# Eddie-Wang1120/Eddie-Wang-Hackathon2023

Measured on AMD Instinct MI355X. Metric: decode tokens/s, whole job (encoder + cross-KV + language-ID + prefill + greedy decode), Whisper large-v2 int8 weight-only + int8 KV; rtf reported beside it, higher is better.
Workload: dtype f16

## Files before the change

eddie-wang-hackathon2023_amd/csrc/attn_encoder.hip:

```cpp
#include <stdlib.h>

#include <type_traits>

#include "common.h"
#include "kernels.h"

namespace wm {

constexpr int KT_KEYS = 64;
constexpr int AROW = 128;
constexpr int KV_TILE = KT_KEYS * AROW;

template <int QB, bool PERSIST = false>
__global__ __launch_bounds__(256, 2) void attn_encoder_kernel(AttnEncParams p) {
    __shared__ __attribute__((aligned(1024))) unsigned char smem[4 * KV_TILE];
    auto sK = [&](int b) { return smem + b * 2 * KV_TILE; };
    auto sV = [&](int b) { return smem + b * 2 * KV_TILE + KV_TILE; };

    const int tid = threadIdx.x, lane = tid & 63, wid = tid >> 6;
    const int g = lane >> 4, li = lane & 15;
    const int C = p.H * 64;
    const int nx = (p.T + 64 * QB - 1) / (64 * QB), n_heads = p.H * p.B;
    const int n_items = 8 * ((n_heads + 7) / 8) * nx;
    int item = blockIdx.x;
    do {
    const int hh = ((item >> 3) / nx) * 8 + (item & 7), bx = (item >> 3) % nx;
    if (hh < n_heads) {
    const int h = hh % p.H, b = hh / p.H;
    const int q_base = bx * (64 * QB) + wid * (16 * QB);
    const h16* base = p.qkv + (size_t)b * p.T * p.ld;

    half8v qf[QB][2];
#pragma unroll
    for (int qb = 0; qb < QB; ++qb) {
        int qrow = q_base + qb * 16 + li;
        if (qrow > p.T - 1) qrow = p.T - 1;
#pragma unroll
        for (int s = 0; s < 2; ++s)
            qf[qb][s] = *(const half8v*)(base + (size_t)qrow * p.ld + h * 64 + s * 32 + g * 8);
    }

    auto load_kv = [&](int tile, int buf) {
#pragma unroll
        for (int i = 0; i < 2; ++i) {
            const int piece = wid + 4 * i;
            const int r = piece * 8 + (lane >> 3);
            int key = tile * KT_KEYS + r;
            if (key > p.T - 1) key = p.T - 1;
            const h16* row = base + (size_t)key * p.ld + h * 64 + (((lane & 7) ^ ((r >> 1) & 7)) * 8);
            __builtin_amdgcn_global_load_lds((const __attribute__((address_space(1))) void*)(row + C),
                                             (__attribute__((address_space(3))) void*)(sK(buf) + piece * 1024), 16, 0, 0);
            __builtin_amdgcn_global_load_lds((const __attribute__((address_space(1))) void*)(row + 2 * C),
                                             (__attribute__((address_space(3))) void*)(sV(buf) + piece * 1024), 16, 0, 0);
        }
    };

    float4v o[4][QB];
#pragma unroll
    for (int db = 0; db < 4; ++db)
#pragma unroll
        for (int qb = 0; qb < QB; ++qb) o[db][qb] = float4v{0.f, 0.f, 0.f, 0.f};
    float m_run[QB], l_run[QB];
#pragma unroll
    for (int qb = 0; qb < QB; ++qb) { m_run[qb] = -INFINITY; l_run[qb] = 0.f; }

    const int ntiles = (p.T + KT_KEYS - 1) / KT_KEYS;
    load_kv(0, 0);
    asm volatile("s_waitcnt vmcnt(0)" ::: "memory");
    __syncthreads();

    const int k_swz = (li >> 1) & 7;
    const int k_off0 = li * AROW + ((g ^ k_swz) << 4), k_off1 = li * AROW + (((g + 4) ^ k_swz) << 4);
    const int v_row = 4 * g + (li >> 2), v_swz = (v_row >> 1) & 7;
    const int v_base = v_row * AROW + (li & 1) * 8, v_chunk = (li & 3) >> 1;

    auto tile_body = [&](int t, auto TAIL_) {
        constexpr bool TAIL = decltype(TAIL_)::value;
        const int cur = t & 1;
        if (t + 1 < ntiles) load_kv(t + 1, cur ^ 1);

        float4v sacc[4][QB];
#pragma unroll
        for (int kb = 0; kb < 4; ++kb) {
            const half8v k0 = *(const half8v*)(sK(cur) + k_off0 + kb * 16 * AROW);
            const half8v k1 = *(const half8v*)(sK(cur) + k_off1 + kb * 16 * AROW);
#pragma unroll
            for (int qb = 0; qb < QB; ++qb) {
                float4v a = float4v{0.f, 0.f, 0.f, 0.f};
                a = __builtin_amdgcn_mfma_f32_16x16x32_f16(k0, qf[qb][0], a, 0, 0, 0);
                a = __builtin_amdgcn_mfma_f32_16x16x32_f16(k1, qf[qb][1], a, 0, 0, 0);
                sacc[kb][qb] = a;
            }
        }
        const int key0 = t * KT_KEYS + 4 * g;
        half8v pf[2][QB];
        constexpr float LOG2E = 1.4426950408889634f;
        float mx[QB];
#pragma unroll
        for (int qb = 0; qb < QB; ++qb) {
            float m = -INFINITY;
#pragma unroll
            for (int kb = 0; kb < 4; ++kb)
#pragma unroll
                for (int r = 0; r < 4; ++r) {
                    if (TAIL && key0 + 16 * kb + r >= p.T) sacc[kb][qb][r] = -INFINITY;
                    m = fmaxf(m, sacc[kb][qb][r]);
                }
            mx[qb] = m;
        }
        {
            float o16[QB];
#pragma unroll
            for (int qb = 0; qb < QB; ++qb) o16[qb] = __shfl_xor(mx[qb], 16);
#pragma unroll
            for (int qb = 0; qb < QB; ++qb) mx[qb] = fmaxf(mx[qb], o16[qb]);
            float o32[QB];
#pragma unroll
            for (int qb = 0; qb < QB; ++qb) o32[qb] = __shfl_xor(mx[qb], 32);
#pragma unroll
            for (int qb = 0; qb < QB; ++qb) mx[qb] = fmaxf(mx[qb], o32[qb]);
        }
        float mL[QB], alpha[QB];
        bool moved = false;
#pragma unroll
        for (int qb = 0; qb < QB; ++qb) {
            const float m_old = m_run[qb];
            const float m_new = fmaxf(m_old, r16(mx[qb]));
            float mn = __fmul_rn(m_new, LOG2E), mo = __fmul_rn(m_old, LOG2E);
            asm volatile("" : "+v"(mn), "+v"(mo));
            mL[qb] = mn;
            alpha[qb] = __builtin_amdgcn_exp2f(__fsub_rn(mo, mL[qb]));
            moved |= (m_new != m_old);
            m_run[qb] = m_new;
        }
        const bool any_moved = __builtin_amdgcn_ballot_w64(moved) != 0;
#pragma unroll
        for (int qb = 0; qb < QB; ++qb) {
            float ps = 0.f;
            const half2v one2 = {(h16)1.0f, (h16)1.0f};
#pragma unroll
            for (int kb = 0; kb < 4; ++kb)
#pragma unroll
                for (int r = 0; r < 4; r += 2) {
                    const half2v s2 = __builtin_convertvector(float2v{sacc[kb][qb][r], sacc[kb][qb][r + 1]}, half2v);
                    const float p0 = __builtin_amdgcn_exp2f(__fmaf_rn((float)s2[0], LOG2E, -mL[qb]));
                    const float p1 = __builtin_amdgcn_exp2f(__fmaf_rn((float)s2[1], LOG2E, -mL[qb]));
                    const half2v p2 = __builtin_convertvector(float2v{p0, p1}, half2v);
                    ps = __builtin_amdgcn_fdot2(p2, one2, ps, false);
                    pf[kb >> 1][qb][(kb & 1) * 4 + r] = p2[0];
                    pf[kb >> 1][qb][(kb & 1) * 4 + r + 1] = p2[1];
                }
            l_run[qb] = __fmaf_rn(l_run[qb], alpha[qb], ps);
        }
        if (any_moved) {
#pragma unroll
            for (int qb = 0; qb < QB; ++qb)
#pragma unroll
                for (int db = 0; db < 4; ++db) o[db][qb] *= alpha[qb];
        }
#pragma unroll
        for (int c = 0; c < 2; ++c) {
#pragma unroll
            for (int db = 0; db < 4; ++db) {
                const unsigned char* va = sV(cur) + v_base + (c * 32) * AROW + (((2 * db + v_chunk) ^ v_swz) << 4);
                const short4r lo = __builtin_amdgcn_ds_read_tr16_b64_v4i16(
                    (__attribute__((address_space(3))) short4r*)(va));
                const short4r hi = __builtin_amdgcn_ds_read_tr16_b64_v4i16(
                    (__attribute__((address_space(3))) short4r*)(va + 16 * AROW));
                half8v vf;
                const half4v l4 = __builtin_bit_cast(half4v, lo), h4 = __builtin_bit_cast(half4v, hi);
#pragma unroll
                for (int j = 0; j < 4; ++j) { vf[j] = l4[j]; vf[4 + j] = h4[j]; }
#pragma unroll
                for (int qb = 0; qb < QB; ++qb)
                    o[db][qb] = __builtin_amdgcn_mfma_f32_16x16x32_f16(vf, pf[c][qb], o[db][qb], 0, 0, 0);
            }
        }
        asm volatile("s_waitcnt vmcnt(0)" ::: "memory");
        __syncthreads();
    };
    for (int t = 0; t + 1 < ntiles; ++t) tile_body(t, std::false_type{});
    if (p.T % KT_KEYS != 0) tile_body(ntiles - 1, std::true_type{}); else tile_body(ntiles - 1, std::false_type{});

#pragma unroll
    for (int qb = 0; qb < QB; ++qb) {
        const int qrow = q_base + qb * 16 + li;
        float l = l_run[qb];
        l += __shfl_xor(l, 16);
        l += __shfl_xor(l, 32);
        if (qrow >= p.T) continue;
        const float inv = 1.0f / l;
        h16* dst = p.out + ((size_t)b * p.T + qrow) * p.ldo + h * 64;
#pragma unroll
        for (int db = 0; db < 4; ++db) {
            half4v w;
#pragma unroll
            for (int r = 0; r < 4; ++r) {
                float t = o[db][qb][r] * inv;
                asm volatile("" : "+v"(t));
                w[r] = (h16)t;
            }
            *(half4v*)(dst + db * 16 + g * 4) = w;
        }
    }
    }
    item += gridDim.x;
    } while (PERSIST && item < n_items);
}

int launch_attn_encoder(const AttnEncParams& p, hipStream_t stream) {
    WM_REQUIRE(p.T >= 1 && p.H >= 1 && p.B >= 1, "attn_encoder: bad shape");
    WM_REQUIRE(p.ld % 8 == 0 && p.ldo % 4 == 0, "attn_encoder: leading dimensions must keep 16-byte alignment");
    static const int lab_wgs = lab_env_int("WM_ATTN_MAX_WGS", 0);
    const int max_wgs = p.max_wgs > 0 ? p.max_wgs : lab_wgs;
    const int heads8 = 8 * ((p.H * p.B + 7) / 8);
    if (p.T > 128 && max_wgs > 0 && max_wgs < ((p.T + 255) / 256) * p.H * p.B) {
        hipLaunchKernelGGL((attn_encoder_kernel<4, true>), dim3(max_wgs >= 8 ? max_wgs / 8 * 8 : max_wgs), dim3(256), 0, stream, p);
    } else if (p.T > 128) {
        hipLaunchKernelGGL(attn_encoder_kernel<4>, dim3(heads8 * ((p.T + 255) / 256)), dim3(256), 0, stream, p);
    } else {
        hipLaunchKernelGGL(attn_encoder_kernel<2>, dim3(heads8 * ((p.T + 127) / 128)), dim3(256), 0, stream, p);
    }
    WM_LAUNCH_CHECK(stream, "attn_encoder");
    return 0;
}

}
```

eddie-wang-hackathon2023_amd/csrc/common.h:

```cpp
#pragma once
#include <hip/hip_runtime.h>
#include <hip/hip_fp16.h>
#include <stdint.h>
#include <stddef.h>

namespace wm {

typedef _Float16 h16;
typedef _Float16 half2v __attribute__((ext_vector_type(2)));
typedef float float2v __attribute__((ext_vector_type(2)));
typedef _Float16 half4v __attribute__((ext_vector_type(4)));
typedef _Float16 half8v __attribute__((ext_vector_type(8)));
typedef float float4v __attribute__((ext_vector_type(4)));
typedef float float16v __attribute__((ext_vector_type(16)));
typedef short short4r __attribute__((__vector_size__(4 * sizeof(short))));
typedef unsigned int u32x4 __attribute__((ext_vector_type(4)));

constexpr int WAVE = 64;

void set_error(const char* fmt, ...);
#define WM_CHECK_HIP(expr)                                                                  \
    do {                                                                                    \
        hipError_t _e = (expr);                                                             \
        if (_e != hipSuccess) {                                                             \
            wm::set_error("%s failed: %s (%s:%d)", #expr, hipGetErrorString(_e), __FILE__,  \
                          __LINE__);                                                        \
            return 2;                                                                       \
        }                                                                                   \
    } while (0)
#define WM_REQUIRE(cond, ...)                                                               \
    do {                                                                                    \
        if (!(cond)) {                                                                      \
            wm::set_error(__VA_ARGS__);                                                     \
            return 1;                                                                       \
        }                                                                                   \
    } while (0)
int post_launch_check(hipStream_t s, const char* what);
#define WM_LAUNCH_CHECK(stream, what)                                                       \
    do {                                                                                    \
        int _r = wm::post_launch_check(stream, what);                                       \
        if (_r) return _r;                                                                  \
    } while (0)

int lab_env_int(const char* name, int dflt);
const char* lab_env_str(const char* name);

__device__ __forceinline__ float mul_rn(float a, float b) {
    float r = a * b;
    asm volatile("" : "+v"(r));
    return r;
}
__device__ __forceinline__ float f32_as_is(float v) {
    asm volatile("" : "+v"(v));
    return v;
}
template <int CTRL>
__device__ __forceinline__ float wave_dpp(float v) {
    return __builtin_bit_cast(float, __builtin_amdgcn_update_dpp(0, __builtin_bit_cast(int, v), CTRL, 0xf, 0xf, true));
}
#define WM_SWAP_GUARD "s_nop 7\n\ts_nop 7\n\ts_nop 2\n\t"
__device__ __forceinline__ void wave_swap32(int& x, int& y) {
    asm volatile(WM_SWAP_GUARD "v_mov_b32 %1, %0\n\ts_nop 1\n\tv_permlane32_swap_b32 %0, %1\n\ts_nop 1" : "+v"(x), "=&v"(y));
}
__device__ __forceinline__ void wave_swap16(int& x, int& y) {
    asm volatile(WM_SWAP_GUARD "v_mov_b32 %1, %0\n\ts_nop 1\n\tv_permlane16_swap_b32 %0, %1\n\ts_nop 1" : "+v"(x), "=&v"(y));
}
__device__ __forceinline__ float wave_add_xor16(float v) { int x = __builtin_bit_cast(int, v), y; wave_swap16(x, y); return __builtin_bit_cast(float, x) + __builtin_bit_cast(float, y); }
__device__ __forceinline__ float wave_add_xor32(float v) { int x = __builtin_bit_cast(int, v), y; wave_swap32(x, y); return __builtin_bit_cast(float, x) + __builtin_bit_cast(float, y); }
__device__ __forceinline__ float wave_max_xor16(float v) { int x = __builtin_bit_cast(int, v), y; wave_swap16(x, y); return fmaxf(__builtin_bit_cast(float, x), __builtin_bit_cast(float, y)); }
__device__ __forceinline__ float wave_max_xor32(float v) { int x = __builtin_bit_cast(int, v), y; wave_swap32(x, y); return fmaxf(__builtin_bit_cast(float, x), __builtin_bit_cast(float, y)); }
__device__ __forceinline__ float wave_sum(float v) {
    int x = __builtin_bit_cast(int, v), y;
    wave_swap32(x, y);
    v = __builtin_bit_cast(float, x) + __builtin_bit_cast(float, y);
    x = __builtin_bit_cast(int, v);
    wave_swap16(x, y);
    v = __builtin_bit_cast(float, x) + __builtin_bit_cast(float, y);
    v += wave_dpp<0x128>(v);
    v += wave_dpp<0x124>(v);
    v += wave_dpp<0x4E>(v);
    v += wave_dpp<0xB1>(v);
    return v;
}
__device__ __forceinline__ float wave_sum_pre_mfma(float v) {
    int x = __builtin_bit_cast(int, v), y;
    asm volatile("v_mov_b32 %1, %0\n\ts_nop 1\n\tv_permlane32_swap_b32 %0, %1\n\ts_nop 1" : "+v"(x), "=&v"(y));
    v = __builtin_bit_cast(float, x) + __builtin_bit_cast(float, y);
    x = __builtin_bit_cast(int, v);
    asm volatile("v_mov_b32 %1, %0\n\ts_nop 1\n\tv_permlane16_swap_b32 %0, %1\n\ts_nop 1" : "+v"(x), "=&v"(y));
    v = __builtin_bit_cast(float, x) + __builtin_bit_cast(float, y);
    v += wave_dpp<0x128>(v);
    v += wave_dpp<0x124>(v);
    v += wave_dpp<0x4E>(v);
    v += wave_dpp<0xB1>(v);
    return v;
}
__device__ __forceinline__ float wave_sum_nomfma(float v) { return wave_sum_pre_mfma(v); }
#define WM_X8_STEP(SWAP)                                                                                                         \
    int x0 = __builtin_bit_cast(int, v[0]), x1 = __builtin_bit_cast(int, v[1]), x2 = __builtin_bit_cast(int, v[2]),              \
        x3 = __builtin_bit_cast(int, v[3]), x4 = __builtin_bit_cast(int, v[4]), x5 = __builtin_bit_cast(int, v[5]),              \
        x6 = __builtin_bit_cast(int, v[6]), x7 = __builtin_bit_cast(int, v[7]), y0, y1, y2, y3, y4, y5, y6, y7;                  \
    asm volatile("v_mov_b32 %8, %0\n\tv_mov_b32 %9, %1\n\tv_mov_b32 %10, %2\n\tv_mov_b32 %11, %3\n\t"                            \
                 "v_mov_b32 %12, %4\n\tv_mov_b32 %13, %5\n\tv_mov_b32 %14, %6\n\tv_mov_b32 %15, %7\n\ts_nop 1\n\t"                   \
                 SWAP " %0, %8\n\t" SWAP " %1, %9\n\t" SWAP " %2, %10\n\t" SWAP " %3, %11\n\t"                                    \
                 SWAP " %4, %12\n\t" SWAP " %5, %13\n\t" SWAP " %6, %14\n\t" SWAP " %7, %15\n\ts_nop 1"                            \
                 : "+v"(x0), "+v"(x1), "+v"(x2), "+v"(x3), "+v"(x4), "+v"(x5), "+v"(x6), "+v"(x7),                               \
                   "=&v"(y0), "=&v"(y1), "=&v"(y2), "=&v"(y3), "=&v"(y4), "=&v"(y5), "=&v"(y6), "=&v"(y7));                      \
    v[0] = __builtin_bit_cast(float, x0) + __builtin_bit_cast(float, y0); v[1] = __builtin_bit_cast(float, x1) + __builtin_bit_cast(float, y1);   \
    v[2] = __builtin_bit_cast(float, x2) + __builtin_bit_cast(float, y2); v[3] = __builtin_bit_cast(float, x3) + __builtin_bit_cast(float, y3);   \
    v[4] = __builtin_bit_cast(float, x4) + __builtin_bit_cast(float, y4); v[5] = __builtin_bit_cast(float, x5) + __builtin_bit_cast(float, y5);   \
    v[6] = __builtin_bit_cast(float, x6) + __builtin_bit_cast(float, y6); v[7] = __builtin_bit_cast(float, x7) + __builtin_bit_cast(float, y7);
__device__ __forceinline__ void wave_add_xor16_x8_nomfma(float* v) { WM_X8_STEP("v_permlane16_swap_b32") }
__device__ __forceinline__ void wave_add_xor32_x8_nomfma(float* v) { WM_X8_STEP("v_permlane32_swap_b32") }
#undef WM_X8_STEP
__device__ __forceinline__ float wave_max_nomfma(float v) {
    int x = __builtin_bit_cast(int, v), y;
    asm volatile("v_mov_b32 %1, %0\n\ts_nop 1\n\tv_permlane32_swap_b32 %0, %1\n\ts_nop 1" : "+v"(x), "=&v"(y));
    v = fmaxf(__builtin_bit_cast(float, x), __builtin_bit_cast(float, y));
    x = __builtin_bit_cast(int, v);
    asm volatile("v_mov_b32 %1, %0\n\ts_nop 1\n\tv_permlane16_swap_b32 %0, %1\n\ts_nop 1" : "+v"(x), "=&v"(y));
    v = fmaxf(__builtin_bit_cast(float, x), __builtin_bit_cast(float, y));
    v = fmaxf(v, wave_dpp<0x128>(v));
    v = fmaxf(v, wave_dpp<0x124>(v));
    v = fmaxf(v, wave_dpp<0x4E>(v));
    v = fmaxf(v, wave_dpp<0xB1>(v));
    return v;
}
__device__ __forceinline__ float wave_max(float v) {
    int x = __builtin_bit_cast(int, v), y;
    wave_swap32(x, y);
    v = fmaxf(__builtin_bit_cast(float, x), __builtin_bit_cast(float, y));
    x = __builtin_bit_cast(int, v);
    wave_swap16(x, y);
    v = fmaxf(__builtin_bit_cast(float, x), __builtin_bit_cast(float, y));
    v = fmaxf(v, wave_dpp<0x128>(v));
    v = fmaxf(v, wave_dpp<0x124>(v));
    v = fmaxf(v, wave_dpp<0x4E>(v));
    v = fmaxf(v, wave_dpp<0xB1>(v));
    return v;
}
__device__ __forceinline__ void lane_rows_swap16(uint32_t& a, uint32_t& b) {
    asm volatile("s_nop 1\n\tv_permlane16_swap_b32 %0, %1\n\ts_nop 1" : "+v"(a), "+v"(b));
}
__device__ __forceinline__ float r16(float x) { return (float)(h16)x; }
__device__ __forceinline__ float r16_f32(float x) { asm("" : "+v"(x)); return (float)(h16)x; }

__device__ __forceinline__ float fast_erf(float x) {
    const float ax = fabsf(x);
    const float t = __builtin_amdgcn_rcpf(1.0f + 0.3275911f * ax);
    const float poly = t * (0.254829592f + t * (-0.284496736f + t * (1.421413741f + t * (-1.453152027f + t * 1.061405429f))));
    const float e = __builtin_amdgcn_exp2f(ax * (ax * -1.4426950408889634f));
    return copysignf(1.0f - poly * e, x);
}
__device__ __forceinline__ float gelu_erf(float x) { return 0.5f * x * (1.0f + fast_erf(x * 0.70710678118654752f)); }
__device__ __forceinline__ float2v gelu_erf2(float2v x) {
    const float2v xs = x * 0.70710678118654752f;
    const float2v ax = {fabsf(xs[0]), fabsf(xs[1])};
    const float2v d = 1.0f + 0.3275911f * ax;
    const float2v t = {__builtin_amdgcn_rcpf(d[0]), __builtin_amdgcn_rcpf(d[1])};
    const float2v poly = t * (0.254829592f + t * (-0.284496736f + t * (1.421413741f + t * (-1.453152027f + t * 1.061405429f))));
    const float2v a2 = ax * (ax * -1.4426950408889634f);
    const float2v e = {__builtin_amdgcn_exp2f(a2[0]), __builtin_amdgcn_exp2f(a2[1])};
    const float2v m = 1.0f - poly * e;
    const float2v erf = {copysignf(m[0], xs[0]), copysignf(m[1], xs[1])};
    return 0.5f * x * (1.0f + erf);
}
__device__ __forceinline__ float gelu_tanh(float x) {
    return 0.5f * x * (1.0f + tanhf(0.7978845608028654f * (x + 0.044715f * x * x * x)));
}

__device__ __forceinline__ void cvt_s8x4_f16x4(uint32_t w, half2v& lo, half2v& hi) {
    uint32_t u = w ^ 0x80808080u;
    uint32_t a = __builtin_amdgcn_perm(0x64646464u, u, 0x07010700u);
    uint32_t b = __builtin_amdgcn_perm(0x64646464u, u, 0x07030702u);
    const half2v k = {(h16)1152.0f, (h16)1152.0f};
    lo = __builtin_bit_cast(half2v, a) - k;
    hi = __builtin_bit_cast(half2v, b) - k;
}

}
```

Measured before the change: 16420.

## Prefetch next persistent item and skip dead tail tiles in encoder attention

Restructures the encoder flash-attention kernel so a persistent workgroup prefetches the next item's Q and first K/V tile during the last tile of the current item, removing the drain-and-reload bubble between items. It also skips MFMA and softmax work for key blocks beyond T in the tail tile and for query blocks beyond T in partial tiles. Shuffle-based row reductions are replaced with permlane16/32 swap inline-asm helpers. This adds template variants and register pressure, and the cross-item double-buffer parity logic is easy to get wrong.

```diff
diff --git a/eddie-wang-hackathon2023_amd/csrc/attn_encoder.hip b/eddie-wang-hackathon2023_amd/csrc/attn_encoder.hip
--- a/eddie-wang-hackathon2023_amd/csrc/attn_encoder.hip
+++ b/eddie-wang-hackathon2023_amd/csrc/attn_encoder.hip
@@ -10,6 +10,11 @@
 constexpr int KT_KEYS = 64;
 constexpr int AROW = 128;
 constexpr int KV_TILE = KT_KEYS * AROW;
+
+#ifndef WM_ATTN_OPT
+#define WM_ATTN_OPT 15
+#endif
+constexpr bool OPT_TAIL = WM_ATTN_OPT & 1, OPT_PARTQ = WM_ATTN_OPT & 2, OPT_SWAP = WM_ATTN_OPT & 4, OPT_NEXT = WM_ATTN_OPT & 8;
 
 template <int QB, bool PERSIST = false>
 __global__ __launch_bounds__(256, 2) void attn_encoder_kernel(AttnEncParams p) {
@@ -22,32 +27,35 @@
     const int C = p.H * 64;
     const int nx = (p.T + 64 * QB - 1) / (64 * QB), n_heads = p.H * p.B;
     const int n_items = 8 * ((n_heads + 7) / 8) * nx;
-    int item = blockIdx.x;
-    do {
-    const int hh = ((item >> 3) / nx) * 8 + (item & 7), bx = (item >> 3) % nx;
-    if (hh < n_heads) {
-    const int h = hh % p.H, b = hh / p.H;
-    const int q_base = bx * (64 * QB) + wid * (16 * QB);
-    const h16* base = p.qkv + (size_t)b * p.T * p.ld;
+    auto head_of = [&](int it) { return ((it >> 3) / nx) * 8 + (it & 7); };
+    auto live_item = [&](int it) {
+        while (it < n_items && head_of(it) >= n_heads) it += gridDim.x;
+        return it;
+    };
+    auto head_cols = [&](int it) { const int hh = head_of(it); return p.qkv + (size_t)(hh / p.H) * p.T * p.ld + (hh % p.H) * 64; };
+    auto query_base = [&](int it) { return ((it >> 3) % nx) * (64 * QB) + wid * (16 * QB); };
 
     half8v qf[QB][2];
-#pragma unroll
-    for (int qb = 0; qb < QB; ++qb) {
-        int qrow = q_base + qb * 16 + li;
-        if (qrow > p.T - 1) qrow = p.T - 1;
-#pragma unroll
-        for (int s = 0; s < 2; ++s)
-            qf[qb][s] = *(const half8v*)(base + (size_t)qrow * p.ld + h * 64 + s * 32 + g * 8);
-    }
-
-    auto load_kv = [&](int tile, int buf) {
+    auto load_q = [&](int it) __attribute__((always_inline)) {
+        const h16* cols = head_cols(it);
+        const int q_base = query_base(it);
+#pragma unroll
+        for (int qb = 0; qb < QB; ++qb) {
+            int qrow = q_base + qb * 16 + li;
+            if (qrow > p.T - 1) qrow = p.T - 1;
+#pragma unroll
+            for (int s = 0; s < 2; ++s)
+                qf[qb][s] = *(const half8v*)(cols + (size_t)qrow * p.ld + s * 32 + g * 8);
+        }
+    };
+    auto load_kv = [&](const h16* cols, int tile, int buf) __attribute__((always_inline)) {
 #pragma unroll
         for (int i = 0; i < 2; ++i) {
             const int piece = wid + 4 * i;
             const int r = piece * 8 + (lane >> 3);
             int key = tile * KT_KEYS + r;
             if (key > p.T - 1) key = p.T - 1;
-            const h16* row = base + (size_t)key * p.ld + h * 64 + (((lane & 7) ^ ((r >> 1) & 7)) * 8);
+            const h16* row = cols + (size_t)key * p.ld + (((lane & 7) ^ ((r >> 1) & 7)) * 8);
             __builtin_amdgcn_global_load_lds((const __attribute__((address_space(1))) void*)(row + C),
                                              (__attribute__((address_space(3))) void*)(sK(buf) + piece * 1024), 16, 0, 0);
             __builtin_amdgcn_global_load_lds((const __attribute__((address_space(1))) void*)(row + 2 * C),
@@ -55,6 +63,21 @@
         }
     };
 
+    const int ntiles = (p.T + KT_KEYS - 1) / KT_KEYS;
+    int item = live_item(blockIdx.x);
+    if (item >= n_items) return;
+    int buf0 = 0;
+    load_q(item);
+    load_kv(head_cols(item), 0, 0);
+    asm volatile("s_waitcnt vmcnt(0)" ::: "memory");
+    __syncthreads();
+    for (;;) {
+    const int next = PERSIST ? live_item(item + gridDim.x) : n_items;
+    const bool has_next = next < n_items;
+    const int hh = head_of(item), h = hh % p.H, b = hh / p.H;
+    const int q_base = query_base(item);
+    const h16* cols = head_cols(item);
+
     float4v o[4][QB];
 #pragma unroll
     for (int db = 0; db < 4; ++db)
@@ -64,34 +87,43 @@
 #pragma unroll
     for (int qb = 0; qb < QB; ++qb) { m_run[qb] = -INFINITY; l_run[qb] = 0.f; }
 
-    const int ntiles = (p.T + KT_KEYS - 1) / KT_KEYS;
-    load_kv(0, 0);
-    asm volatile("s_waitcnt vmcnt(0)" ::: "memory");
-    __syncthreads();
 
     const int k_swz = (li >> 1) & 7;
     const int k_off0 = li * AROW + ((g ^ k_swz) << 4), k_off1 = li * AROW + (((g + 4) ^ k_swz) << 4);
     const int v_row = 4 * g + (li >> 2), v_swz = (v_row >> 1) & 7;
     const int v_base = v_row * AROW + (li & 1) * 8, v_chunk = (li & 3) >> 1;
 
-    auto tile_body = [&](int t, auto TAIL_) {
+    const int tail = p.T - (ntiles - 1) * KT_KEYS;
+    const int n_kb = (tail + 15) >> 4, n_c = (tail + 31) >> 5;
+    const int nq_raw = (p.T - q_base + 15) >> 4, nq = nq_raw < 0 ? 0 : nq_raw < QB ? nq_raw : QB;
+
+    auto tile_body = [&](int t, auto TAIL_, auto PARTQ_, auto LAST_) __attribute__((always_inline)) {
         constexpr bool TAIL = decltype(TAIL_)::value;
-        const int cur = t & 1;
-        if (t + 1 < ntiles) load_kv(t + 1, cur ^ 1);
+        constexpr bool LAST = decltype(LAST_)::value && PERSIST && OPT_NEXT;
+        constexpr bool PARTQ = decltype(PARTQ_)::value;
+        auto live_kb = [&](int kb) { return !(TAIL && OPT_TAIL) || kb < n_kb; };
+        auto live_qb = [&](int qb) { return !PARTQ || qb < nq; };
+        const int cur = (buf0 + t) & 1;
+        if (t + 1 < ntiles) load_kv(cols, t + 1, cur ^ 1);
+        if (LAST && has_next) load_kv(head_cols(next), 0, cur ^ 1);
+        if (!PARTQ || nq > 0) {
 
         float4v sacc[4][QB];
 #pragma unroll
         for (int kb = 0; kb < 4; ++kb) {
+            if (!live_kb(kb)) continue;
             const half8v k0 = *(const half8v*)(sK(cur) + k_off0 + kb * 16 * AROW);
             const half8v k1 = *(const half8v*)(sK(cur) + k_off1 + kb * 16 * AROW);
 #pragma unroll
             for (int qb = 0; qb < QB; ++qb) {
+                if (!live_qb(qb)) continue;
                 float4v a = float4v{0.f, 0.f, 0.f, 0.f};
                 a = __builtin_amdgcn_mfma_f32_16x16x32_f16(k0, qf[qb][0], a, 0, 0, 0);
                 a = __builtin_amdgcn_mfma_f32_16x16x32_f16(k1, qf[qb][1], a, 0, 0, 0);
                 sacc[kb][qb] = a;
             }
         }
+        if (LAST && has_next) load_q(next);
         const int key0 = t * KT_KEYS + 4 * g;
         half8v pf[2][QB];
         constexpr float LOG2E = 1.4426950408889634f;
@@ -99,16 +131,23 @@
 #pragma unroll
         for (int qb = 0; qb < QB; ++qb) {
             float m = -INFINITY;
-#pragma unroll
-            for (int kb = 0; kb < 4; ++kb)
+            if (live_qb(qb)) {
+#pragma unroll
+            for (int kb = 0; kb < 4; ++kb) {
+                if (!live_kb(kb)) continue;
 #pragma unroll
                 for (int r = 0; r < 4; ++r) {
                     if (TAIL && key0 + 16 * kb + r >= p.T) sacc[kb][qb][r] = -INFINITY;
                     m = fmaxf(m, sacc[kb][qb][r]);
                 }
+            }
+            }
             mx[qb] = m;
         }
-        {
+        if constexpr (OPT_SWAP) {
+            lane_xor_step<QB, true, false>(mx);
+            lane_xor_step<QB, false, false>(mx);
+        } else {
             float o16[QB];
 #pragma unroll
             for (int qb = 0; qb < QB; ++qb) o16[qb] = __shfl_xor(mx[qb], 16);
@@ -124,6 +163,7 @@
         bool moved = false;
 #pragma unroll
         for (int qb = 0; qb < QB; ++qb) {
+            if (!live_qb(qb)) continue;
             const float m_old = m_run[qb];
             const float m_new = fmaxf(m_old, r16(mx[qb]));
             float mn = __fmul_rn(m_new, LOG2E), mo = __fmul_rn(m_old, LOG2E);
@@ -136,10 +176,16 @@
         const bool any_moved = __builtin_amdgcn_ballot_w64(moved) != 0;
 #pragma unroll
         for (int qb = 0; qb < QB; ++qb) {
+            if (!live_qb(qb)) continue;
             float ps = 0.f;
             const half2v one2 = {(h16)1.0f, (h16)1.0f};
 #pragma unroll
-            for (int kb = 0; kb < 4; ++kb)
+            for (int kb = 0; kb < 4; ++kb) {
+                if (!live_kb(kb)) {
+#pragma unroll
+                    for (int r = 0; r < 4; ++r) pf[kb >> 1][qb][(kb & 1) * 4 + r] = (h16)0.0f;
+                    continue;
+                }
 #pragma unroll
                 for (int r = 0; r < 4; r += 2) {
                     const half2v s2 = __builtin_convertvector(float2v{sacc[kb][qb][r], sacc[kb][qb][r + 1]}, half2v);
@@ -150,16 +196,20 @@
                     pf[kb >> 1][qb][(kb & 1) * 4 + r] = p2[0];
                     pf[kb >> 1][qb][(kb & 1) * 4 + r + 1] = p2[1];
                 }
+            }
             l_run[qb] = __fmaf_rn(l_run[qb], alpha[qb], ps);
         }
         if (any_moved) {
 #pragma unroll
-            for (int qb = 0; qb < QB; ++qb)
+            for (int qb = 0; qb < QB; ++qb) {
+                if (!live_qb(qb)) continue;
 #pragma unroll
                 for (int db = 0; db < 4; ++db) o[db][qb] *= alpha[qb];
+            }
         }
 #pragma unroll
         for (int c = 0; c < 2; ++c) {
+            if (TAIL && OPT_TAIL && c >= n_c) continue;
 #pragma unroll
             for (int db = 0; db < 4; ++db) {
                 const unsigned char* va = sV(cur) + v_base + (c * 32) * AROW + (((2 * db + v_chunk) ^ v_swz) << 4);
@@ -172,24 +222,39 @@
 #pragma unroll
                 for (int j = 0; j < 4; ++j) { vf[j] = l4[j]; vf[4 + j] = h4[j]; }
 #pragma unroll
-                for (int qb = 0; qb < QB; ++qb)
+                for (int qb = 0; qb < QB; ++qb) {
+                    if (!live_qb(qb)) continue;
                     o[db][qb] = __builtin_amdgcn_mfma_f32_16x16x32_f16(vf, pf[c][qb], o[db][qb], 0, 0, 0);
-            }
-        }
+                }
+            }
+        }
+        }
+        if (LAST && PARTQ && has_next && nq == 0) load_q(next);
         asm volatile("s_waitcnt vmcnt(0)" ::: "memory");
         __syncthreads();
     };
-    for (int t = 0; t + 1 < ntiles; ++t) tile_body(t, std::false_type{});
-    if (p.T % KT_KEYS != 0) tile_body(ntiles - 1, std::true_type{}); else tile_body(ntiles - 1, std::false_type{});
-
+    auto all_tiles = [&](auto PARTQ_) __attribute__((always_inline)) {
+        for (int t = 0; t + 1 < ntiles; ++t) tile_body(t, std::false_type{}, PARTQ_, std::false_type{});
+        if (p.T % KT_KEYS != 0) tile_body(ntiles - 1, std::true_type{}, PARTQ_, std::true_type{});
+        else tile_body(ntiles - 1, std::false_type{}, PARTQ_, std::true_type{});
+    };
+    if (!OPT_PARTQ || nq == QB) all_tiles(std::false_type{}); else all_tiles(std::true_type{});
+
+    if constexpr (OPT_SWAP) {
+        lane_xor_step<QB, true, true>(l_run);
+        lane_xor_step<QB, false, true>(l_run);
+    } else {
+#pragma unroll
+        for (int qb = 0; qb < QB; ++qb) {
+            l_run[qb] += __shfl_xor(l_run[qb], 16);
+            l_run[qb] += __shfl_xor(l_run[qb], 32);
+        }
+    }
 #pragma unroll
     for (int qb = 0; qb < QB; ++qb) {
         const int qrow = q_base + qb * 16 + li;
-        float l = l_run[qb];
-        l += __shfl_xor(l, 16);
-        l += __shfl_xor(l, 32);
         if (qrow >= p.T) continue;
-        const float inv = 1.0f / l;
+        const float inv = 1.0f / l_run[qb];
         h16* dst = p.out + ((size_t)b * p.T + qrow) * p.ldo + h * 64;
 #pragma unroll
         for (int db = 0; db < 4; ++db) {
@@ -203,9 +268,18 @@
             *(half4v*)(dst + db * 16 + g * 4) = w;
         }
     }
-    }
-    item += gridDim.x;
-    } while (PERSIST && item < n_items);
+    if (!has_next) break;
+    item = next;
+    if (PERSIST && OPT_NEXT) {
+        buf0 = (buf0 + ntiles) & 1;
+    } else {
+        buf0 = 0;
+        load_q(item);
+        load_kv(head_cols(item), 0, 0);
+        asm volatile("s_waitcnt vmcnt(0)" ::: "memory");
+        __syncthreads();
+    }
+    }
 }
 
 int launch_attn_encoder(const AttnEncParams& p, hipStream_t stream) {
diff --git a/eddie-wang-hackathon2023_amd/csrc/common.h b/eddie-wang-hackathon2023_amd/csrc/common.h
--- a/eddie-wang-hackathon2023_amd/csrc/common.h
+++ b/eddie-wang-hackathon2023_amd/csrc/common.h
@@ -142,6 +142,43 @@
 __device__ __forceinline__ void lane_rows_swap16(uint32_t& a, uint32_t& b) {
     asm volatile("s_nop 1\n\tv_permlane16_swap_b32 %0, %1\n\ts_nop 1" : "+v"(a), "+v"(b));
 }
+#define WM_SWAP4(INS) "s_nop 1\n\t" INS " %0, %4\n\t" INS " %1, %5\n\t" INS " %2, %6\n\t" INS " %3, %7\n\ts_nop 1"
+#define WM_SWAP2(INS) "s_nop 1\n\t" INS " %0, %2\n\t" INS " %1, %3\n\ts_nop 1"
+#define WM_MAX4 "\n\tv_max_f32 %0, %0, %4\n\tv_max_f32 %1, %1, %5\n\tv_max_f32 %2, %2, %6\n\tv_max_f32 %3, %3, %7"
+#define WM_MAX2 "\n\tv_max_f32 %0, %0, %2\n\tv_max_f32 %1, %1, %3"
+#define WM_OPS4 : "+v"(a[0]), "+v"(a[1]), "+v"(a[2]), "+v"(a[3]), "+v"(b[0]), "+v"(b[1]), "+v"(b[2]), "+v"(b[3])
+#define WM_OPS2 : "+v"(a[0]), "+v"(a[1]), "+v"(b[0]), "+v"(b[1])
+template <int N, bool ROWS16, bool SUM>
+__device__ __forceinline__ void lane_swap_pairs(uint32_t (&a)[N], uint32_t (&b)[N]) {
+    static_assert(N == 2 || N == 4, "lane_swap_pairs: 2 or 4 values");
+    if constexpr (N == 4) {
+        if constexpr (ROWS16 && SUM) asm volatile(WM_SWAP4("v_permlane16_swap_b32") WM_OPS4);
+        else if constexpr (ROWS16) asm volatile(WM_SWAP4("v_permlane16_swap_b32") WM_MAX4 WM_OPS4);
+        else if constexpr (SUM) asm volatile(WM_SWAP4("v_permlane32_swap_b32") WM_OPS4);
+        else asm volatile(WM_SWAP4("v_permlane32_swap_b32") WM_MAX4 WM_OPS4);
+    } else {
+        if constexpr (ROWS16 && SUM) asm volatile(WM_SWAP2("v_permlane16_swap_b32") WM_OPS2);
+        else if constexpr (ROWS16) asm volatile(WM_SWAP2("v_permlane16_swap_b32") WM_MAX2 WM_OPS2);
+        else if constexpr (SUM) asm volatile(WM_SWAP2("v_permlane32_swap_b32") WM_OPS2);
+        else asm volatile(WM_SWAP2("v_permlane32_swap_b32") WM_MAX2 WM_OPS2);
+    }
+}
+#undef WM_SWAP4
+#undef WM_SWAP2
+#undef WM_MAX4
+#undef WM_MAX2
+#undef WM_OPS4
+#undef WM_OPS2
+template <int N, bool ROWS16, bool SUM>
+__device__ __forceinline__ void lane_xor_step(float (&v)[N]) {
+    uint32_t a[N], b[N];
+#pragma unroll
+    for (int i = 0; i < N; ++i) a[i] = b[i] = __builtin_bit_cast(uint32_t, v[i]);
+    lane_swap_pairs<N, ROWS16, SUM>(a, b);
+#pragma unroll
+    for (int i = 0; i < N; ++i)
+        v[i] = SUM ? __builtin_bit_cast(float, a[i]) + __builtin_bit_cast(float, b[i]) : __builtin_bit_cast(float, a[i]);
+}
 __device__ __forceinline__ float r16(float x) { return (float)(h16)x; }
 __device__ __forceinline__ float r16_f32(float x) { asm("" : "+v"(x)); return (float)(h16)x; }
 
```

Result: faster. 16620 (median of 6 runs) (+1.2%).
